# sj-shoff/ImageProcessor

Hardware: AMD Instinct MI355X
Metric: images/sec (resize+thumb+watermark) on 1080p batch at 1/2/4/8 MI355X (higher is better)
Workload: dtype f32+f64

## Files before the change

imageprocessor_amd/build.py:

```python
import concurrent.futures as cf
import os
import subprocess
import sys

HERE = os.path.dirname(os.path.abspath(__file__))
CSRC = os.path.join(HERE, "csrc")
OBJ = os.path.join(HERE, "build")
LIB = os.path.join(HERE, "libipx.so")
SOURCES = ["ipx_kernels.hip", "ipx_ks_generic.hip", "ipx_ks_fused.hip", "ipx_ks_tail.hip", "ipx_jpeg.hip", "ipx_jpeg_entropy.hip", "ipx_jpeg_dec.hip", "ipx_jpeg_dec_par.hip", "ipx_runtime.hip", "ipx_jpeg_runtime.hip", "ipx_pool.hip", "ipx_gif.hip", "ipx_gif_dec.hip", "ipx_png.hip", "ipx_png_dec.hip", "ipx_host.cpp", "ipx_ks_host.cpp", "ipx_batcher.cpp", "ipx_ops.cpp", "ipx_font.cpp", "ipx_jpeg_host.cpp", "ipx_jpeg_dec_host.cpp", "ipx_jpeg_dec_prog.cpp", "ipx_gif_host.cpp", "ipx_gif_dec_host.cpp", "ipx_png_host.cpp", "ipx_png_dec_host.cpp"]
HEADERS = ["ipx_internal.h", "ipx_runtime_internal.h", "ipx_device.h", "ipx_ks.h", "ipx_ks_exact.h", "ipx_threads.h", "ipx_batcher.h", "ipx_pool_core.h", "ipx_gif.h", "ipx_gif_dec.h", "ipx_png.h", "ipx_png_dec.h", os.path.join("..", "..", "include", "ipx.h")]
FLAGS = ["-O3", "-std=c++17", "-fPIC", "--offload-arch=gfx950", "-ffp-contract=off",
         "-fno-fast-math", "-Wall", "-Wno-unused-function"] + os.environ.get("IPX_CXXFLAGS", "").split()


def hipcc():
    for c in (os.environ.get("HIPCC"), "/opt/rocm/bin/hipcc", "hipcc"):
        if c and (os.path.isabs(c) and os.path.exists(c) or not os.path.isabs(c)):
            return c
    return "hipcc"


def sources():
    return [f for f in SOURCES if os.path.exists(os.path.join(CSRC, f))]


def _obj(src):
    return os.path.join(OBJ, src + ".o")


def _newest_header():
    return max(os.path.getmtime(os.path.join(CSRC, h)) for h in HEADERS if os.path.exists(os.path.join(CSRC, h)))


def _stale_objects(force):
    hdr = _newest_header()
    out = []
    for f in sources():
        o = _obj(f)
        if force or not os.path.exists(o) or os.path.getmtime(o) < max(hdr, os.path.getmtime(os.path.join(CSRC, f))):
            out.append(f)
    return out


def stale():
    if not os.path.exists(LIB):
        return True
    t = os.path.getmtime(LIB)
    return any(os.path.getmtime(os.path.join(CSRC, f)) > t for f in sources() + HEADERS if os.path.exists(os.path.join(CSRC, f)))


def build(force=False, verbose=False, jobs=None):
    if not force and not stale():
        return LIB
    os.makedirs(OBJ, exist_ok=True)
    todo = _stale_objects(force)

    def compile_one(f):
        cmd = [hipcc()] + FLAGS + ["-c", "-o", _obj(f), os.path.join(CSRC, f)]
        if verbose:
            print(" ".join(cmd), flush=True)
        subprocess.check_call(cmd)

    jobs = jobs or max(1, min(len(todo), (os.cpu_count() or 2)))
    if todo:
        with cf.ThreadPoolExecutor(jobs) as ex:
            list(ex.map(compile_one, todo))
    cmd = [hipcc(), "-shared", "-fPIC", "--offload-arch=gfx950", "-o", LIB] + [_obj(f) for f in sources()]
    if verbose:
        print(" ".join(cmd), flush=True)
    subprocess.check_call(cmd)
    return LIB


if __name__ == "__main__":
    build(force="--force" in sys.argv, verbose=True)
    print(LIB)
```

imageprocessor_amd/csrc/ipx_ks.h:

```cpp
#pragma once

#include <vector>

#include "ipx_internal.h"

namespace ipx {

struct KsAxis {
    int dw = 0, sw = 0;
    int ntap = 0;
    std::vector<int32_t> lo, cnt;
    std::vector<double> w;
    std::vector<double> itw, itwffff;
    std::vector<double> ones;
};
bool ks_build_axis(int dw, int sw, KsAxis *out);

struct KsAxisDev {
    const int32_t *lo, *cnt;
    const double *w, *itw, *itwffff, *ones;
    int ntap;
};
size_t ks_axis_bytes(const KsAxis &a);
void ks_axis_pack(const KsAxis &a, uint8_t *h, const uint8_t *d, KsAxisDev *out);

enum {
    IPX_SRC_RGBA_CROP = 8,
    IPX_SRC_NRGBA_CROP = 9,
    IPX_SRC_YCBCR_CROP = 10,
    IPX_SRC_TAP64_CROP = 11
};
inline int ks_crop_kind(int kind)
{
    return kind == IPX_SRC_NRGBA ? IPX_SRC_NRGBA_CROP : kind == IPX_SRC_YCBCR ? IPX_SRC_YCBCR_CROP : kind == IPX_SRC_TAP64 ? IPX_SRC_TAP64_CROP
                                                                                                                           : IPX_SRC_RGBA_CROP;
}

struct KsGenArgs {
    uint8_t *dst; int dstride; size_t dst_fs;
    int dr_x0, dr_y0;
    int adr_x0, adr_y0, adr_x1, adr_y1;
    int sr_x0, sr_y0;
    KsAxisDev ax, ay;
    int op;
    const int *opaque_flag;
    int kind;
    const uint8_t *src; int sstride; size_t src_fs;
    const uint8_t *cb, *cr; int cstride, ratio; size_t c_fs;
    int nframes;
    int src_w;
};
hipError_t launch_ks_generic(const KsGenArgs &a, hipStream_t s);

}

namespace ipx {

struct KsStrip { int c0, c1, t0, tw; };
struct KsSeg { int ys, r0, r1; };
template <int NACC> struct KsRowT { double w[NACC], itw[NACC], ones[NACC]; int32_t emit[NACC]; float wf[NACC]; };
static_assert(sizeof(KsRowT<2>) == 64 && sizeof(KsRowT<4>) == 128, "row entries are copied dword-wise");

struct KsFusedOut {
    uint8_t *out; size_t frame_stride; int ostride, obytes;
    int dw, dh, sr_x0, sr_y0;
    int kind;
    int mode, aone;
    int pk;
    int ntap;
    int waves, cpl;
    int wcols;
    const double *wx;
    const float *wxf;
    int split, ntapf;
    float feps;
    const double *itwf;
    const int32_t *xlo;
    const int32_t *colb;
    const void *rows;
    const int32_t *rowoff;
};
struct KsFusedArgs {
    const uint8_t *src; size_t src_fs; int sstride, sw, sh;
    int src_kind;
    int taps_le_alpha;
    const uint8_t *cb, *cr; int cstride, ratio; size_t c_fs;
    uint8_t *wm; size_t wm_fs; int wm_stride;
    int nframes, nstrips, nseg, nthreads, pitch, dbuf;
    const KsStrip *strips; const KsSeg *segs;
    int nout; KsFusedOut o[2];
    int lds_w[2], lds_rows, lds_open;
    int open_per_wave;
    uint8_t wave_role[16];
    unsigned long long *stamps;
    int *redo;
    uint2 *fix; int *fix_count; int fix_cap[2], fix_stride;
};
struct KsText { const DevGlyph *gl; int n; Rect bbox; uint32_t sr, sg, sb, sa; };
struct KsFix { uint2 *list = nullptr; int *count = nullptr; int cap[2] = {0, 0}; KsAxisDev ax[2], ay[2]; };
struct KsFusedGeom { int nseg = 0; const KsSeg *segs = nullptr; const void *rows[2] = {nullptr, nullptr}; const int32_t *rowoff[2] = {nullptr, nullptr}; };
struct KsFusedPlan {
    bool ok = false;
    int nacc = 2, rows = 4, pitch = 0, nstrips = 0, nthreads = 0, nstg = 0, dbuf = 0;
    int lds_w[2] = {0, 0}, lds_rows = 0, lds_open = 0, lds_bytes = 0;
    struct Lds { int dbuf = 0, lds_w[2] = {0, 0}, lds_rows = 0, lds_open = 0, open_per_wave = 0, lds_bytes = 0; } fast;
    const KsStrip *strips = nullptr;
    struct Out { int ntap = 0, waves = 0, cpl = 0, wcols = 0; const double *wx = nullptr, *itwf = nullptr; const int32_t *xlo = nullptr, *colb = nullptr;
                 const float *wxf = nullptr; float feps = 0; int split = 1, ntapf = 0; } o[2];
    KsFusedGeom whole, split;
};
constexpr int kKsSplitRows = 96;
constexpr int kKsRows = 4;
constexpr int kKsMaxStage = 3;
constexpr int kKsMaxWaves = 12;
constexpr int kKsMaxThreads = 64 * kKsMaxWaves;
constexpr int kKsMaxCpl = 2;
constexpr int kKsSplitTaps = 16;
constexpr int kKsOpenPerWave = 128;
struct KsFusedIn { int dw, dh, sr_x0, sr_y0; const KsAxis *hx, *hy; int top_taps = 0; };
bool ks_fused_plan(int sw, int sh, const KsFusedIn *sc0, const KsFusedIn *sc1, int px_bytes, std::vector<uint8_t> *blob, KsFusedPlan *out);
void ks_fused_rebase(KsFusedPlan *p, const uint8_t *dev_blob);
hipError_t launch_ks_fused(const KsFusedPlan &p, KsFusedArgs &a, const KsFix *fix, const KsText *text, int cus, hipStream_t s, bool *matched, bool *text_done);
hipError_t launch_ks_fix(const KsGenArgs &g, const uint2 *list, size_t list_stride, const int *count, int count_stride, int cap, hipStream_t s);

struct KsTailArgs {
    KsGenArgs g[2];
    const uint2 *list[2]; const int *count[2]; int cap[2];
    size_t list_stride; int count_stride;
    int nframes;
    int R[2], chunks[2];
    uint8_t *wm; int wm_stride; size_t wm_fs;
    KsText text;
    int tbx, tby;
};
hipError_t launch_ks_tail(KsTailArgs t, hipStream_t s);

}
```

imageprocessor_amd/csrc/ipx_ks_tail.hip:

```cpp
#include <algorithm>
#include <cstdlib>

#include "ipx_ks_exact.h"

namespace ipx {
namespace {

constexpr int kTailThreads = 256;
constexpr int kTextRows = 4;

template <int KIND>
__device__ __forceinline__ void tail_exact(KsGenArgs a, const uint2 *list, size_t list_stride, const int *count, int count_stride, int cap, int R,
                                           int frame, int chunk, int chunks)
{
    const int n = min(count[(size_t)frame * count_stride], cap);
    list += (size_t)frame * list_stride;
    a.dst += frame * a.dst_fs;
    a.src += frame * a.src_fs;
    if (KIND == IPX_SRC_YCBCR || KIND == IPX_SRC_YCBCR_CROP) { a.cb += frame * a.c_fs; a.cr += frame * a.c_fs; }
    const int lane = (int)threadIdx.x & 63, wv = (int)threadIdx.x >> 6;
    const int per_wave = 64 / R, sub = lane / R, sl = lane - sub * R, per_block = (kTailThreads >> 6) * per_wave;
    ks_exact_list<KIND>(a, list, n, chunk * per_block, chunks * per_block, wv * per_wave + sub, R, sub, sl);
}

__device__ __forceinline__ void tail_text(const KsTailArgs &t, DevGlyph *tab, int f, int rb)
{
    const int by = rb / t.tbx, bx = rb - by * t.tbx;
    const Rect bbox = t.text.bbox;
    const int n = t.text.n;
    const int x = bbox.x0 + bx * 64 + ((int)threadIdx.x & 63);
    const int ybase = bbox.y0 + by * (4 * kTextRows) + ((int)threadIdx.x >> 6);
    uint8_t *frame = t.wm + (size_t)f * t.wm_fs;
    uint32_t d[kTextRows][1], d0[kTextRows];
#pragma unroll
    for (int r = 0; r < kTextRows; r++) {
        const int y = ybase + 4 * r;
        d0[r] = d[r][0] = x < bbox.x1 && y < bbox.y1 ? *(const uint32_t *)(frame + (size_t)y * t.wm_stride + (size_t)x * 4) : 0u;
    }
    for (int g = (int)threadIdx.x; g < n; g += kTailThreads) tab[g] = t.text.gl[g];
    __syncthreads();
    glyph_walk<1, kTextRows, 4>(tab, n, x, ybase, bbox, d, t.text.sr, t.text.sg, t.text.sb, t.text.sa);
#pragma unroll
    for (int r = 0; r < kTextRows; r++) {
        const int y = ybase + 4 * r;
        if (x < bbox.x1 && y < bbox.y1 && d[r][0] != d0[r]) *(uint32_t *)(frame + (size_t)y * t.wm_stride + (size_t)x * 4) = d[r][0];
    }
}

template <int K0, int K1>
__global__ __launch_bounds__(kTailThreads) void ks_tail_kernel(KsTailArgs t)
{
    __shared__ DevGlyph tab[kMaxGlyphs];
    const int nx = t.chunks[0] + t.chunks[1], per = nx + t.tbx * t.tby, b = (int)blockIdx.x;
    const int frame = b / per, c = b - frame * per;
    if (c < nx) {
        const int k = c >= t.chunks[0] ? 1 : 0, chunk = c - (k ? t.chunks[0] : 0);
        if (K0 == K1 || k == 0)
            tail_exact<K0>(k ? t.g[1] : t.g[0], t.list[k], t.list_stride, t.count[k], t.count_stride, t.cap[k], t.R[k], frame, chunk, t.chunks[k]);
        else
            tail_exact<K1>(t.g[1], t.list[1], t.list_stride, t.count[1], t.count_stride, t.cap[1], t.R[1], frame, chunk, t.chunks[1]);
        return;
    }
    tail_text(t, tab, frame, c - nx);
}

template <int K0, int K1>
void tail_go(const KsTailArgs &t, unsigned blocks, hipStream_t s)
{
    hipLaunchKernelGGL((ks_tail_kernel<K0, K1>), dim3(blocks), dim3(kTailThreads), 0, s, t);
}

template <int S, int C>
bool tail_pair(int k0, int k1, const KsTailArgs &t, unsigned blocks, hipStream_t s)
{
    if (k0 == S && k1 == S) tail_go<S, S>(t, blocks, s);
    else if (k0 == S && k1 == C) tail_go<S, C>(t, blocks, s);
    else if (k0 == C && k1 == C) tail_go<C, C>(t, blocks, s);
    else return false;
    return true;
}

}

hipError_t launch_ks_tail(KsTailArgs t, hipStream_t s)
{
    if (t.nframes <= 0) return hipSuccess;
    const char *ev = getenv("IPX_KS_TAIL_BLOCKS");
    const int budget = ev && atoi(ev) > 0 ? atoi(ev) : 2048;
    for (int k = 0; k < 2; k++) {
        t.R[k] = 8; t.chunks[k] = 0;
        if (!t.list[k] || t.cap[k] <= 0) { t.cap[k] = 0; continue; }
        const int ntap = t.g[k].ay.ntap;
        t.R[k] = ntap <= 4 ? 4 : ntap <= 8 ? 8 : ntap <= 16 ? 16 : 64;
        const int per_block = (kTailThreads / 64) * (64 / t.R[k]), most = (t.cap[k] + per_block - 1) / per_block;
        t.chunks[k] = std::max(1, std::min(most, std::max(1, budget / t.nframes)));
    }
    const bool text = t.wm && t.text.gl && t.text.n > 0 && !t.text.bbox.empty();
    if (!text) t.text.n = 0;
    t.tbx = text ? (t.text.bbox.dx() + 63) / 64 : 0;
    t.tby = text ? (t.text.bbox.dy() + 4 * kTextRows - 1) / (4 * kTextRows) : 0;
    const long long blocks = (long long)t.nframes * (t.chunks[0] + t.chunks[1]) + (long long)t.nframes * t.tbx * t.tby;
    if (blocks <= 0) return hipSuccess;
    if (blocks > 0x7fffffffLL) return hipErrorInvalidValue;
    const int k0 = t.chunks[0] ? t.g[0].kind : t.g[1].kind, k1 = t.chunks[1] ? t.g[1].kind : k0;
    const bool none = !t.chunks[0] && !t.chunks[1];
    if (none) { tail_go<IPX_SRC_RGBA, IPX_SRC_RGBA>(t, (unsigned)blocks, s); return hipGetLastError(); }
    if (!tail_pair<IPX_SRC_RGBA, IPX_SRC_RGBA_CROP>(k0, k1, t, (unsigned)blocks, s) && !tail_pair<IPX_SRC_NRGBA, IPX_SRC_NRGBA_CROP>(k0, k1, t, (unsigned)blocks, s) &&
        !tail_pair<IPX_SRC_YCBCR, IPX_SRC_YCBCR_CROP>(k0, k1, t, (unsigned)blocks, s) && !tail_pair<IPX_SRC_TAP64, IPX_SRC_TAP64_CROP>(k0, k1, t, (unsigned)blocks, s))
        return hipErrorInvalidValue;
    return hipGetLastError();
}

}
```

imageprocessor_amd/csrc/ipx_runtime.hip:

```cpp
#include <algorithm>
#include <chrono>
#include <condition_variable>
#include <cstdlib>
#include <cstring>
#include <map>
#include <mutex>
#include <new>
#include <thread>
#include <utility>
#include <vector>

#include "ipx_runtime_internal.h"
#include "ipx_ks.h"

#ifndef IPX_DIAG
#define IPX_DIAG 0
#endif

namespace {

struct ScalePrep {
    bool empty;
    Rect adr;
};
// ... 47 lines not shown
    int cstride = 0, ratio = 0;
    int w = 0, h = 0;
    int nframes = 1;
    size_t frame_stride = 0, c_frame_stride = 0;
    bool le_alpha = false;
};

int dev_draw_src(hipStream_t s, uint8_t *dst, int dw, int dh, int dstride, Rect r, const DevSrc &src, int spx,
                 int spy, int op, size_t dst_fs = 0)
{
    if (op != IPX_OP_OVER && op != IPX_OP_SRC) { set_error("draw: unknown op %d", op); return IPX_ERR_INVALID; }
    int mx = 0, my = 0;
    if (!draw_clip(r, dw, dh, true, src.w, src.h, spx, spy, false, 0, 0, mx, my)) return IPX_OK;
    uint8_t *d = dst + (size_t)r.y0 * dstride + (size_t)r.x0 * 4;
    if (src.kind == IPX_SRC_YCBCR)
        IPX_HIP(launch_draw_ycbcr(d, dstride, src.pix, src.stride, src.cb, src.cr, src.cstride, src.ratio, spx, spy,
                                  r.dx(), r.dy(), s, src.nframes, dst_fs, src.frame_stride, src.c_frame_stride));
    else if (src.kind == IPX_SRC_NRGBA)
        IPX_HIP(launch_draw_nrgba(d, dstride, src.pix + (size_t)spy * src.stride + (size_t)spx * 4, src.stride, r.dx(),
                                  r.dy(), op, s, src.nframes, dst_fs, src.frame_stride));
    else if (src.kind == IPX_SRC_TAP64)
        IPX_HIP(launch_draw_tap64(d, dstride, src.pix + (size_t)spy * src.stride + (size_t)spx * 8, src.stride, r.dx(), r.dy(), op, s,
                                  src.nframes, dst_fs, src.frame_stride));
    else
        for (int i = 0; i < std::max(1, src.nframes); i++)
            IPX_HIP(launch_draw(d + (size_t)i * dst_fs, dstride, src.pix + (size_t)i * src.frame_stride + (size_t)spy * src.stride + (size_t)spx * 4,
                                src.stride, r.dx(), r.dy(), op, s));
    return IPX_OK;
}

int dev_scale_src(ipx_ctx *ctx, hipStream_t s, int *flag, uint8_t *dst, int dw, int dh, int dstride, const Rect &dr,
                  const DevSrc &src, const Rect &sr, int op, size_t dst_fs = 0, int kind_override = -1, const KsAxisDev *axes = nullptr)
{
    ScalePrep pr;
    int rc = scale_prepare(dw, dh, dr, src.w, src.h, sr, op, &pr);
    if (rc) return rc;
    if (pr.empty) return IPX_OK;
    if (src.kind == IPX_SRC_YCBCR) op = IPX_OP_SRC;
    if (op == IPX_OP_OVER && src.kind == IPX_SRC_TAP64) IPX_HIP(launch_opaque_scan_tap64(src.pix, src.w, src.h, src.stride, flag, s));
    else if (op == IPX_OP_OVER) IPX_HIP(launch_opaque_scan(src.pix, src.w, src.h, src.stride, flag, s));
    KsGenArgs a{};
    if (axes) { a.ax = axes[0]; a.ay = axes[1]; }
    else {
        if ((rc = ks_axis_get(ctx, dr.dx(), sr.dx(), &a.ax))) return rc;
        if ((rc = ks_axis_get(ctx, dr.dy(), sr.dy(), &a.ay))) return rc;
    }
    a.dst = dst; a.dstride = dstride; a.src = src.pix; a.sstride = src.stride;
    a.dr_x0 = dr.x0; a.dr_y0 = dr.y0;
    a.adr_x0 = pr.adr.x0; a.adr_y0 = pr.adr.y0; a.adr_x1 = pr.adr.x1; a.adr_y1 = pr.adr.y1;
    a.sr_x0 = sr.x0; a.sr_y0 = sr.y0;
    a.op = op; a.opaque_flag = op == IPX_OP_OVER ? flag : nullptr;
    a.kind = kind_override >= 0 ? kind_override : src.kind;
    a.cb = src.cb; a.cr = src.cr; a.cstride = src.cstride; a.ratio = src.ratio;
    a.nframes = src.nframes; a.src_fs = src.frame_stride; a.c_fs = src.c_frame_stride; a.dst_fs = dst_fs;
    IPX_HIP(launch_ks_generic(a, s));
    return IPX_OK;
}

DevSrc rgba_src(const uint8_t *p, int w, int h, int stride, int kind = IPX_SRC_RGBA)
{
    DevSrc d;
    d.kind = kind; d.pix = p; d.stride = stride; d.w = w; d.h = h;
    return d;
}

int dev_draw(hipStream_t s, uint8_t *dst, int dw, int dh, int dstride, Rect r, const uint8_t *src,
             int sw, int sh, int sstride, int spx, int spy, int op)
{
    return dev_draw_src(s, dst, dw, dh, dstride, r, rgba_src(src, sw, sh, sstride), spx, spy, op);
}

int dev_scale(ipx_ctx *ctx, hipStream_t s, int *flag, uint8_t *dst, int dw, int dh, int dstride, const Rect &dr,
              const uint8_t *src, int sw, int sh, int sstride, const Rect &sr, int op)
{
    return dev_scale_src(ctx, s, flag, dst, dw, dh, dstride, dr, rgba_src(src, sw, sh, sstride), sr, op);
}

int glyphs_for_frame(const ipx_glyphset *gs, int dw, int dh, ClippedGlyphs *out)
{
    std::lock_guard<std::mutex> lk(gs->mu);
    auto it = gs->clipped.find({dw, dh});
    if (it != gs->clipped.end()) { *out = it->second; return IPX_OK; }
    std::vector<DevGlyph> tab;
    Rect bb{0, 0, 0, 0};
    for (const GlyphHost &g : gs->g) {
        Rect r = g.dr;
        int spx = 0, spy = 0, mpx = g.mpx, mpy = g.mpy;
        if (!draw_clip(r, dw, dh, false, 0, 0, spx, spy, true, g.mw, g.mh, mpx, mpy)) continue;
        DevGlyph d;
        d.mask = gs->masks_dev + g.mask_off + (size_t)mpy * g.mw + mpx;
        d.mstride = g.mw;
        d.x0 = r.x0; d.y0 = r.y0; d.x1 = r.x1; d.y1 = r.y1;
        if (tab.empty()) bb = r;
        else {
            bb.x0 = std::min(bb.x0, r.x0); bb.y0 = std::min(bb.y0, r.y0);
            bb.x1 = std::max(bb.x1, r.x1); bb.y1 = std::max(bb.y1, r.y1);
        }
        tab.push_back(d);
    }
    ClippedGlyphs c;
    c.n = (int)tab.size();
    c.bbox = bb;
    if (c.n) {
        IPX_HIP(hipMalloc((void **)&c.dev, tab.size() * sizeof(DevGlyph)));
        IPX_HIP(hipMemcpy(c.dev, tab.data(), tab.size() * sizeof(DevGlyph), hipMemcpyHostToDevice));
    }
    gs->clipped[{dw, dh}] = c;
    *out = c;
    return IPX_OK;
}

int dev_composite(hipStream_t s, uint8_t *dst, int dw, int dh, int dstride, size_t frame_stride,
                  int nframes, const ipx_glyphset *gs)
{
    ClippedGlyphs c;
    int rc = glyphs_for_frame(gs, dw, dh, &c);
    if (rc) return rc;
    IPX_HIP(launch_composite(dst, dstride, frame_stride, nframes, c.dev, c.n, c.bbox,
                             gs->col[0] * 0x101u, gs->col[1] * 0x101u, gs->col[2] * 0x101u,
                             gs->col[3] * 0x101u, s));
    return IPX_OK;
}

}

extern "C" {

static void prepare_hip_env();
int ipx_device_count(void) try
{
    prepare_hip_env();
    clear_error();
    int n = 0;
    hipError_t e = hipGetDeviceCount(&n);
    if (e != hipSuccess) { (void)hipGetLastError(); set_error("hipGetDeviceCount: %s", hipGetErrorString(e)); return IPX_ERR_NODEVICE; }
    return n;
}
IPX_CATCH_STATUS

static void prepare_hip_env()
{
    static std::once_flag once;
    std::call_once(once, [] {
        if (!getenv("GPU_MAX_HW_QUEUES")) {
            char v[16];
            snprintf(v, sizeof v, "%d", std::max(8, env_int("IPX_LANES", 5) + 3));
            setenv("GPU_MAX_HW_QUEUES", v, 0);
        }
    });
}

int ipx_create(const ipx_config *cfg, ipx_ctx **out) try
{
    clear_error();
    if (!out) { set_error("ipx_create: null out"); return IPX_ERR_INVALID; }
    *out = nullptr;
    prepare_hip_env();
    int ndev = 0;
    if (hipGetDeviceCount(&ndev) != hipSuccess || ndev <= 0) {
        (void)hipGetLastError();
        set_error("no HIP device visible: the pixel path has no CPU fallback");
        return IPX_ERR_NODEVICE;
    }
    int dev = cfg ? cfg->device : -1;
    if (dev < 0) dev = env_int("IPX_DEVICE", env_int("LOCAL_RANK", 0) % ndev);
    if (dev >= ndev) { set_error("device %d out of range (%d visible)", dev, ndev); return IPX_ERR_INVALID; }
    IPX_HIP(hipSetDevice(dev));
    hipDeviceProp_t prop;
    IPX_HIP(hipGetDeviceProperties(&prop, dev));
    if (strncmp(prop.gcnArchName, "gfx950", 6) != 0) {
        set_error("device %d is %s; libipx carries gfx950 code only", dev, prop.gcnArchName);
        return IPX_ERR_NODEVICE;
    }
    ipx_ctx *c = new (std::nothrow) ipx_ctx;
    if (!c) { set_error("out of memory"); return IPX_ERR_NOMEM; }
    c->device = dev;
    c->cus = prop.multiProcessorCount > 0 ? prop.multiProcessorCount : 256;
    int lanes = cfg && cfg->lanes > 0 ? cfg->lanes : env_int("IPX_LANES", 5);
    c->lane_bytes = cfg && cfg->lane_bytes ? cfg->lane_bytes : (size_t)64 << 20;
    c->host_cache_limit = (size_t)std::max(0, env_int("IPX_HOST_CACHE_MB", 8192)) << 20;
    c->lanes.resize(lanes);
    int prio_lo = 0, prio_hi = 0;
    (void)hipDeviceGetStreamPriorityRange(&prio_lo, &prio_hi);
    hipError_t e = hipSuccess;
    if (c->lanes.size() >= 3) e = hipStreamCreateWithPriority(&c->lanes.back().stream, hipStreamNonBlocking, prio_hi);
    if (e == hipSuccess) e = hipStreamCreateWithFlags(&c->stream, hipStreamNonBlocking);
    for (size_t i = 0; i < c->lanes.size(); i++) {
        Lane &l = c->lanes[i];
// ... 281 lines not shown
    if (hipEventCreate(&ev) != hipSuccess) { (void)hipGetLastError(); set_error("hipEventCreate failed"); return nullptr; }
    return ev;
}

int ipx_event_record(ipx_ctx *ctx, void *event, void *stream) try
{
    IPX_ENTER(ctx);
    if (!event) { set_error("ipx_event_record: null event"); return IPX_ERR_INVALID; }
    IPX_HIP(hipEventRecord((hipEvent_t)event, stream ? (hipStream_t)stream : ctx->stream));
    return IPX_OK;
}
IPX_CATCH_STATUS

int ipx_event_elapsed_ms(ipx_ctx *ctx, void *start, void *stop, float *ms) try
{
    IPX_ENTER(ctx);
    if (!start || !stop || !ms) { set_error("ipx_event_elapsed_ms: bad argument"); return IPX_ERR_INVALID; }
    IPX_HIP(hipEventSynchronize((hipEvent_t)stop));
    IPX_HIP(hipEventElapsedTime(ms, (hipEvent_t)start, (hipEvent_t)stop));
    return IPX_OK;
}
IPX_CATCH_STATUS

void ipx_event_destroy(ipx_ctx *ctx, void *event)
{
    if (!ctx || !event) return;
    (void)hipSetDevice(ctx->device);
    (void)hipEventDestroy((hipEvent_t)event);
}

int ipx_dev_scale_bilinear_rgba8(ipx_ctx *ctx, void *stream, uint8_t *dst, int dw, int dh,
                                 int dstride, ipx_rect dr, const uint8_t *src, int sw, int sh,
                                 int sstride, ipx_rect sr, int op) try
{
    IPX_ENTER(ctx);
    IPX_FRAME("ipx_dev_scale_bilinear_rgba8", "destination", dst, dw, dh, dstride);
    IPX_FRAME("ipx_dev_scale_bilinear_rgba8", "source", src, sw, sh, sstride);
    hipStream_t s = stream ? (hipStream_t)stream : ctx->stream;
    AsyncFree mem{s, {}};
    int *flag = nullptr;
    if (op == IPX_OP_OVER) IPX_HIP(mem.get(&flag, sizeof(int)));
    return dev_scale(ctx, s, flag, dst, dw, dh, dstride, to_rect(dr), src, sw, sh, sstride, to_rect(sr), op);
}
IPX_CATCH_STATUS

int ipx_dev_draw_rgba8(ipx_ctx *ctx, void *stream, uint8_t *dst, int dw, int dh, int dstride,
                       ipx_rect r, const uint8_t *src, int sw, int sh, int sstride, int spx, int spy,
                       int op) try
{
    IPX_ENTER(ctx);
    IPX_FRAME("ipx_dev_draw_rgba8", "destination", dst, dw, dh, dstride);
    IPX_FRAME("ipx_dev_draw_rgba8", "source", src, sw, sh, sstride);
    return dev_draw(stream ? (hipStream_t)stream : ctx->stream, dst, dw, dh, dstride, to_rect(r), src,
                    sw, sh, sstride, spx, spy, op);
}
IPX_CATCH_STATUS

int ipx_glyphset_create(ipx_ctx *ctx, const ipx_glyph *glyphs, int n, const uint8_t col[4],
                        ipx_glyphset **out) try
{
    IPX_ENTER(ctx);
    if (!out || n < 0 || (n && !glyphs) || !col) { set_error("ipx_glyphset_create: bad argument"); return IPX_ERR_INVALID; }
    if (n > kMaxGlyphs) { set_error("ipx_glyphset_create: %d glyphs exceed the limit of %d", n, kMaxGlyphs); return IPX_ERR_UNSUPPORTED; }
    *out = nullptr;
    ipx_glyphset *gs = new (std::nothrow) ipx_glyphset;
    if (!gs) { set_error("out of memory"); return IPX_ERR_NOMEM; }
    gs->device = ctx->device;
    memcpy(gs->col, col, 4);
    std::vector<uint8_t> blob;
    for (int i = 0; i < n; i++) {
        const ipx_glyph &g = glyphs[i];
        if (g.mw < 0 || g.mh < 0 || (g.mw && g.mh && (!g.mask || g.mstride < g.mw))) {
            set_error("ipx_glyphset_create: glyph %d has a bad mask", i);
            delete gs;
            return IPX_ERR_INVALID;
        }
        GlyphHost h;
        h.mask_off = blob.size();
        h.mw = g.mw; h.mh = g.mh; h.dr = to_rect(g.dr); h.mpx = g.mpx; h.mpy = g.mpy;
        for (int y = 0; y < g.mh; y++) blob.insert(blob.end(), g.mask + (size_t)y * g.mstride, g.mask + (size_t)y * g.mstride + g.mw);
        gs->g.push_back(h);
    }
    gs->masks_bytes = blob.size();
    if (!blob.empty()) {
        hipError_t e = hipMalloc((void **)&gs->masks_dev, blob.size());
        if (e == hipSuccess) e = hipMemcpy(gs->masks_dev, blob.data(), blob.size(), hipMemcpyHostToDevice);
        if (e != hipSuccess) {
            set_error("glyph mask upload failed: %s", hipGetErrorString(e));
            ipx_glyphset_destroy(ctx, gs);
            return IPX_ERR_HIP;
        }
    }
    *out = gs;
    return IPX_OK;
}
IPX_CATCH_STATUS

void ipx_glyphset_destroy(ipx_ctx *ctx, ipx_glyphset *gs)
{
    if (!gs) return;
    (void)hipSetDevice(ctx ? ctx->device : gs->device);
    for (auto &kv : gs->clipped) if (kv.second.dev) (void)hipFree(kv.second.dev);
    if (gs->masks_dev) (void)hipFree(gs->masks_dev);
    delete gs;
}

int ipx_dev_composite_glyphs_rgba8(ipx_ctx *ctx, void *stream, uint8_t *dst, int dw, int dh,
                                   int dstride, const ipx_glyphset *gs) try
{
    IPX_ENTER(ctx);
    if (!gs) { set_error("ipx_dev_composite_glyphs_rgba8: bad argument"); return IPX_ERR_INVALID; }
    IPX_FRAME("ipx_dev_composite_glyphs_rgba8", "destination", dst, dw, dh, dstride);
    return dev_composite(stream ? (hipStream_t)stream : ctx->stream, dst, dw, dh, dstride, 0, 1, gs);
}
IPX_CATCH_STATUS

int ipx_scale_bilinear_rgba8(ipx_ctx *ctx, uint8_t *dst, int dw, int dh, int dstride, ipx_rect dr,
                             const uint8_t *src, int sw, int sh, int sstride, ipx_rect sr, int op) try
{
    IPX_ENTER(ctx);
    IPX_FRAME("ipx_scale_bilinear_rgba8", "destination", dst, dw, dh, dstride);
    IPX_FRAME("ipx_scale_bilinear_rgba8", "source", src, sw, sh, sstride);
    ScalePrep pr;
    int rc = scale_prepare(dw, dh, to_rect(dr), sw, sh, to_rect(sr), op, &pr);
    if (rc) return rc;
    if (pr.empty || dw == 0 || dh == 0) return IPX_OK;
    LaneLease lane(ctx);
    const size_t sbytes = align256((size_t)sw * sh * 4), dbytes = align256((size_t)dw * dh * 4);
    rc = lane_reserve(lane.get(), sbytes + dbytes);
    if (rc) return rc;
    uint8_t *dsrc = lane->dev, *ddst = lane->dev + sbytes;
    hipStream_t s = lane->stream;
    if (sw && sh) IPX_HIP(hipMemcpy2DAsync(dsrc, (size_t)sw * 4, src, sstride, (size_t)sw * 4, sh, hipMemcpyHostToDevice, s));
    IPX_HIP(hipMemcpy2DAsync(ddst, (size_t)dw * 4, dst, dstride, (size_t)dw * 4, dh, hipMemcpyHostToDevice, s));
    rc = dev_scale(ctx, s, lane->flag, ddst, dw, dh, dw * 4, to_rect(dr), dsrc, sw, sh, sw * 4, to_rect(sr), op);
    if (rc) { (void)hipStreamSynchronize(s); return rc; }
    IPX_HIP(hipMemcpy2DAsync(dst, dstride, ddst, (size_t)dw * 4, (size_t)dw * 4, dh, hipMemcpyDeviceToHost, s));
    IPX_HIP(hipStreamSynchronize(s));
    return IPX_OK;
}
IPX_CATCH_STATUS

int ipx_draw_rgba8(ipx_ctx *ctx, uint8_t *dst, int dw, int dh, int dstride, ipx_rect r,
                   const uint8_t *src, int sw, int sh, int sstride, int spx, int spy, int op) try
{
    IPX_ENTER(ctx);
    IPX_FRAME("ipx_draw_rgba8", "destination", dst, dw, dh, dstride);
    IPX_FRAME("ipx_draw_rgba8", "source", src, sw, sh, sstride);
    if (op != IPX_OP_OVER && op != IPX_OP_SRC) { set_error("draw: unknown op %d", op); return IPX_ERR_INVALID; }
    if (!dw || !dh || !sw || !sh) return IPX_OK;
    LaneLease lane(ctx);
    const size_t sbytes = align256((size_t)sw * sh * 4), dbytes = align256((size_t)dw * dh * 4);
    int rc = lane_reserve(lane.get(), sbytes + dbytes);
    if (rc) return rc;
    uint8_t *dsrc = lane->dev, *ddst = lane->dev + sbytes;
    hipStream_t s = lane->stream;
    IPX_HIP(hipMemcpy2DAsync(dsrc, (size_t)sw * 4, src, sstride, (size_t)sw * 4, sh, hipMemcpyHostToDevice, s));
    IPX_HIP(hipMemcpy2DAsync(ddst, (size_t)dw * 4, dst, dstride, (size_t)dw * 4, dh, hipMemcpyHostToDevice, s));
    rc = dev_draw(s, ddst, dw, dh, dw * 4, to_rect(r), dsrc, sw, sh, sw * 4, spx, spy, op);
    if (rc) { (void)hipStreamSynchronize(s); return rc; }
    IPX_HIP(hipMemcpy2DAsync(dst, dstride, ddst, (size_t)dw * 4, (size_t)dw * 4, dh, hipMemcpyDeviceToHost, s));
    IPX_HIP(hipStreamSynchronize(s));
    return IPX_OK;
}
IPX_CATCH_STATUS

int ipx_composite_glyphs_rgba8(ipx_ctx *ctx, uint8_t *dst, int dw, int dh, int dstride,
                               const ipx_glyph *glyphs, int n, const uint8_t col[4]) try
{
    IPX_ENTER(ctx);
    if (n < 0 || (n && !glyphs) || !col) { set_error("ipx_composite_glyphs_rgba8: bad argument"); return IPX_ERR_INVALID; }
    IPX_FRAME("ipx_composite_glyphs_rgba8", "destination", dst, dw, dh, dstride);
    if (!n || !dw || !dh) return IPX_OK;
    ipx_glyphset *gs = nullptr;
    int rc = ipx_glyphset_create(ctx, glyphs, n, col, &gs);
    if (rc) return rc;
    {
        LaneLease lane(ctx);
        rc = lane_reserve(lane.get(), align256((size_t)dw * dh * 4));
        hipStream_t s = lane->stream;
        hipError_t e = hipSuccess;
        if (!rc) {
            e = hipMemcpy2DAsync(lane->dev, (size_t)dw * 4, dst, dstride, (size_t)dw * 4, dh, hipMemcpyHostToDevice, s);
            if (e == hipSuccess) rc = dev_composite(s, lane->dev, dw, dh, dw * 4, 0, 1, gs);
            if (e == hipSuccess && !rc)
// ... 376 lines not shown
{
    clear_error();
    if (!plan || !info) { set_error("ipx_plan_query: bad argument"); return IPX_ERR_INVALID; }
    *info = plan->info;
    return IPX_OK;
}
IPX_CATCH_STATUS

}

static hipError_t composite_text(const ipx_plan *pl, uint8_t *wm, size_t wm_frame_stride, int n, hipStream_t s)
{
    if (!wm || pl->glyphs.n <= 0 || !pl->p.glyphs) return hipSuccess;
    const uint8_t *c = pl->p.glyphs->col;
    return launch_composite(wm, pl->p.sw * 4, wm_frame_stride, n, pl->glyphs.dev, pl->glyphs.n, pl->glyphs.bbox, c[0] * 0x101u, c[1] * 0x101u,
                            c[2] * 0x101u, c[3] * 0x101u, s);
}

static int run_dev_any(ipx_ctx *ctx, hipStream_t s, const ipx_plan *pl, int n, const DevSrc &src, uint8_t *resize_out, size_t resize_frame_stride,
                       uint8_t *thumb_out, size_t thumb_frame_stride, uint8_t *wm_out, size_t wm_frame_stride)
{
    const int sw = pl->p.sw, sh = pl->p.sh;
    uint8_t *outs[2] = {pl->sc[0].on ? resize_out : nullptr, pl->sc[1].on ? thumb_out : nullptr};
    const size_t ostr[2] = {resize_frame_stride, thumb_frame_stride};
    uint8_t *wm = pl->p.do_watermark ? wm_out : nullptr;
    for (int k = 0; k < 2; k++)
        if (pl->sc[k].dw <= 0 || pl->sc[k].dh <= 0) outs[k] = nullptr;
    if (!wm && !outs[0] && !outs[1]) return IPX_OK;
    int kinds[2] = {src.kind, pl->p.crop_to_fit ? ks_crop_kind(src.kind) : src.kind};

    const bool gray = src.kind == IPX_SRC_YCBCR && src.cstride == 0;
    const KsFusedPlan &fp = pl->fused[src.kind == IPX_SRC_RGBA ? 0 : gray ? 2 : 1];
    if (fp.ok && env_int("IPX_FUSED", 1)) {
        KsFusedArgs a{};
        a.src = src.pix; a.src_fs = src.frame_stride; a.sstride = src.stride; a.sw = sw; a.sh = sh;
        a.src_kind = src.kind; a.cb = src.cb; a.cr = src.cr; a.cstride = src.cstride; a.ratio = src.ratio; a.c_fs = src.c_frame_stride;
        a.wm = wm; a.wm_fs = wm_frame_stride; a.wm_stride = sw * 4;
        a.nframes = n;
        a.taps_le_alpha = src.le_alpha;
        for (int k = 0; k < 2; k++) {
            if (!outs[k]) continue;
            const PlanScale &ps = pl->sc[k];
            KsFusedOut &o = a.o[a.nout++];
            o.out = outs[k]; o.frame_stride = ostr[k]; o.ostride = ps.dw * 4; o.obytes = ps.dw * ps.dh * 4;
            o.dw = ps.dw; o.dh = ps.dh; o.sr_x0 = ps.sr.x0; o.sr_y0 = ps.sr.y0;
            o.kind = kinds[k]; o.pk = k;
        }
        AsyncFree mem{s, {}};
        int *redo = nullptr;
        KsFix fixv, *fix = nullptr;
        const int max_items = n * fp.nstrips * std::max(fp.whole.nseg, fp.split.nseg);
        const bool spec = src.kind == IPX_SRC_RGBA && env_int("IPX_KS_SPEC", 1);
        const bool fast = (spec || src.kind == IPX_SRC_YCBCR || src.kind == IPX_SRC_NRGBA || (src.kind == IPX_SRC_TAP64 && src.le_alpha)) &&
                          env_int("IPX_KS_FAST", 1) != 0;
        if (spec || fast) {
            const int cap_env = env_int("IPX_KS_FIX_CAP", 0);
            int cap[2] = {0, 0};
            for (int k = 0; k < 2; k++)
                if (fast && outs[k]) cap[k] = cap_env > 0 ? cap_env : (int)std::min<size_t>(std::max<size_t>((size_t)pl->sc[k].dw * pl->sc[k].dh / 96, 256), (size_t)1 << 20);
            const size_t flags = align256((size_t)max_items * sizeof(int)), counts = fast ? align256((size_t)n * 2 * sizeof(int)) : 0;
            IPX_HIP(mem.get(&redo, flags + counts + (size_t)n * (cap[0] + cap[1]) * sizeof(uint2)));
            if (fast) {
                fixv.count = (int *)((uint8_t *)redo + flags);
                fixv.list = (uint2 *)((uint8_t *)redo + flags + counts);
                fixv.cap[0] = cap[0]; fixv.cap[1] = cap[1];
                for (int k = 0; k < 2; k++) { fixv.ax[k] = pl->sc[k].ax[0]; fixv.ay[k] = pl->sc[k].ax[1]; }
                IPX_HIP(hipMemsetAsync(fixv.count, 0, (size_t)n * 2 * sizeof(int), s));
                fix = &fixv;
            }
        }
        a.redo = redo;
#if IPX_DIAG
        static unsigned long long *stamp_buf = nullptr;
        if (env_int("IPX_STAMPS", 0)) {
            if (!stamp_buf) IPX_HIP(hipMalloc((void **)&stamp_buf, 24 * sizeof(unsigned long long)));
            IPX_HIP(hipMemsetAsync(stamp_buf, 0, 24 * sizeof(unsigned long long), s));
            a.stamps = stamp_buf;
        }
#endif
        KsText text{}, *txt = nullptr;
        if (wm && pl->glyphs.n > 0 && pl->p.glyphs) {
            const uint8_t *c = pl->p.glyphs->col;
            text = KsText{pl->glyphs.dev, pl->glyphs.n, pl->glyphs.bbox, c[0] * 0x101u, c[1] * 0x101u, c[2] * 0x101u, c[3] * 0x101u};
            txt = &text;
        }
        bool matched = false, text_done = false;
        hipError_t e = launch_ks_fused(fp, a, fix, txt, ctx->cus, s, &matched, &text_done);
        if (fix && matched && e == hipSuccess && env_int("IPX_KS_STATS", 0)) {
            std::vector<int> cnt((size_t)n * 2), flags((size_t)max_items);
            (void)hipMemcpyAsync(cnt.data(), fixv.count, cnt.size() * sizeof(int), hipMemcpyDeviceToHost, s);
            (void)hipMemcpyAsync(flags.data(), redo, flags.size() * sizeof(int), hipMemcpyDeviceToHost, s);
            (void)hipStreamSynchronize(s);
            long long tot[2] = {0, 0}; int mx[2] = {0, 0}, nredo = 0;
            for (int i = 0; i < n; i++) for (int k = 0; k < 2; k++) { tot[k] += cnt[2 * i + k]; mx[k] = std::max(mx[k], cnt[2 * i + k]); }
            for (int f : flags) nredo += f != 0;
            fprintf(stderr, "[ipx ks stats] %d frames: undecided pixels per frame resize mean %.1f max %d (room %d), thumbnail mean %.1f max %d (room %d); %d of %d items redone in float64\n", n,
                    (double)tot[0] / n, mx[0], fixv.cap[0], (double)tot[1] / n, mx[1], fixv.cap[1], nredo, max_items);
        }
#if IPX_DIAG
        if (a.stamps && matched) {
            unsigned long long h[24];
            IPX_HIP(hipMemcpyAsync(h, a.stamps, sizeof h, hipMemcpyDeviceToHost, s));
            IPX_HIP(hipStreamSynchronize(s));
            const char *who[3] = {"resize waves", "thumbnail waves", "idle waves"};
            for (int r = 0; r < 3; r++) {
                double tot = 0;
                for (int i = 0; i < 6; i++) tot += (double)h[r * 8 + i];
                if (tot > 0)
                    fprintf(stderr, "[ipx stamps] %-16s share of wave time: wait-loads %.1f%%  drain %.1f%%  barrier %.1f%%  issue %.1f%%  scaleX %.1f%%  scaleY %.1f%%  (%.3g cycles)\n", who[r],
                            100 * h[r * 8] / tot, 100 * h[r * 8 + 1] / tot, 100 * h[r * 8 + 2] / tot, 100 * h[r * 8 + 3] / tot, 100 * h[r * 8 + 4] / tot, 100 * h[r * 8 + 5] / tot, tot);
            }
        }
#endif
        if (e != hipSuccess) { set_error("one-pass kernel launch failed: %s", hipGetErrorString(e)); return IPX_ERR_HIP; }
        if (matched) {
            if (!text_done) IPX_HIP(composite_text(pl, wm, wm_frame_stride, n, s));
            return IPX_OK;
        }
    }

    if (wm) {
        const int rc = dev_draw_src(s, wm, sw, sh, sw * 4, Rect{0, 0, sw, sh}, src, 0, 0, IPX_OP_SRC, wm_frame_stride);
        if (rc) return rc;
        IPX_HIP(composite_text(pl, wm, wm_frame_stride, n, s));
    }
    for (int k = 0; k < 2; k++) {
        if (!outs[k]) continue;
        const PlanScale &ps = pl->sc[k];
        const int rc = dev_scale_src(ctx, s, nullptr, outs[k], ps.dw, ps.dh, ps.dw * 4, Rect{0, 0, ps.dw, ps.dh}, src, ps.sr, IPX_OP_SRC, ostr[k],
                                     kinds[k], ps.ax);
        if (rc) return rc;
    }
    return IPX_OK;
}


int src_check(const char *who, const ipx_plan *pl, const BatchSrc &b, int n, bool in_hbm)
{
    if (b.type < 0 || b.type >= kSrcTypes) { set_error("%s: unknown source type", who); return IPX_ERR_INVALID; }
    const int bpp = src_bpp(b.type);
    bool ok = pl && n >= 0 && b.plane[0] && (long long)b.stride[0] >= (long long)pl->p.sw * bpp;
    if (ok && b.type == kSrcYCbCr) {
        int cw = 0, ch = 0;
        chroma_size(b.ratio, pl->p.sw, pl->p.sh, &cw, &ch);
        ok = b.plane[1] && b.plane[2] && b.ratio >= 0 && b.ratio <= IPX_YCBCR_440 && b.stride[1] >= cw;
    }
    if (ok && b.type == kSrcPaletted) ok = b.palettes && !(in_hbm && ((uintptr_t)b.palettes & 3));
    if (ok && in_hbm && b.type >= kSrcNRGBA64)
        ok = !(((uintptr_t)b.plane[0] | (uintptr_t)b.stride[0] | b.frame_stride[0]) & (b.type == kSrcCMYK ? 3 : 1));
    if (!ok) { set_error("%s: bad argument", who); return IPX_ERR_INVALID; }
    const int sw = pl->p.sw, sh = pl->p.sh;
    if (!frame_span_ok(sw, sh, b.stride[0], bpp) || (b.type == kSrcYCbCr && !frame_span_ok(sw, sh, b.stride[1], 1)) ||
        (b.type >= kSrcNRGBA64 && !frame_span_ok(sw, sh, (long long)sw * 8, 8))) {
        set_error("%s: %dx%d frames with row strides of %d / %d bytes are beyond the 2 GiB span the kernels address", who, sw, sh, b.stride[0], b.stride[1]);
        return IPX_ERR_UNSUPPORTED;
    }
    if (in_hbm && n > 65535) { set_error("%s: at most 65535 frames per call", who); return IPX_ERR_UNSUPPORTED; }
    return IPX_OK;
}

SrcLayout src_layout(const ipx_plan *pl, const BatchSrc &b, size_t (*frame_rule)(size_t))
{
    SrcLayout L{};
    int cw = 0, ch = 0;
    if (b.type == kSrcYCbCr) chroma_size(b.ratio, pl->p.sw, pl->p.sh, &cw, &ch);
    L.planes = b.type == kSrcYCbCr ? 3 : 1;
    L.row[0] = (size_t)pl->p.sw * src_bpp(b.type); L.h[0] = pl->p.sh; L.fs[0] = frame_rule(L.row[0] * L.h[0]);
    L.row[1] = cw; L.h[1] = ch; L.fs[1] = frame_rule((size_t)cw * ch);
    L.pal = b.type == kSrcPaletted ? 1024 : 0;
    return L;
}

hipError_t src_upload(const BatchSrc &host, const SrcLayout &L, int i0, int m, uint8_t *scratch, int slots, hipStream_t s, const CopyPolicy &cp,
                      BatchSrc *in_hbm)
{
    *in_hbm = host;
    hipError_t e = hipSuccess;
    uint8_t *d = scratch;
    for (int p = 0; p < L.planes && e == hipSuccess; p++) {
        const int k = p ? 1 : 0;
// ... 381 lines not shown
```

imageprocessor_amd/csrc/ipx_runtime_internal.h:

```cpp
#pragma once

#include <sched.h>

#include <algorithm>
#include <cctype>
#include <cstdio>
#include <condition_variable>
#include <cstdlib>
#include <cstring>
#include <deque>
#include <map>
#include <mutex>
#include <string>
#include <utility>
#include <vector>

#include "ipx_internal.h"
#include "ipx_ks.h"

using namespace ipx;

struct Lane {
    hipStream_t stream = nullptr;
    uint8_t *dev = nullptr;
    size_t dev_bytes = 0;
    int *flag = nullptr;
    uint8_t *dec = nullptr;
    size_t dec_bytes = 0;
    uint8_t *pin = nullptr;
    size_t pin_bytes = 0;
    hipEvent_t ev[3] = {nullptr, nullptr, nullptr};
    bool busy = false;
};

struct ipx_ctx {
    int device = 0;
    int cus = 256;
    hipStream_t stream = nullptr;
    std::vector<Lane> lanes;
    size_t lane_bytes = 0;
    std::mutex mu;
    std::condition_variable cv;
    std::mutex host_mu;
    std::map<void *, size_t> host_size;
    std::multimap<size_t, void *> host_free_blocks;
    std::deque<void *> host_lru;
    size_t host_cached = 0, host_cache_limit = (size_t)8 << 30;
    int jj_active = 0;
    uint8_t *flat_chroma = nullptr;
    std::mutex plan_mu;
    std::map<std::string, std::pair<ipx_glyphset *, ipx_plan *>> plan_cache;
    uint64_t plan_clock = 0;
    std::mutex ks_mu;
    std::map<std::pair<int, int>, std::pair<uint8_t *, KsAxisDev>> ks_axes;
    static constexpr size_t kFlatChromaBytes = (size_t)64 << 10;
};

struct GlyphHost {
    size_t mask_off;
    int mw, mh;
    Rect dr;
    int mpx, mpy;
};

struct ClippedGlyphs {
    DevGlyph *dev = nullptr;
    int n = 0;
    Rect bbox{0, 0, 0, 0};
};

struct ipx_glyphset {
    int device = 0;
    std::vector<GlyphHost> g;
    uint8_t *masks_dev = nullptr;
    size_t masks_bytes = 0;
    uint8_t col[4] = {0, 0, 0, 0};
    mutable std::mutex mu;
    mutable std::map<std::pair<int, int>, ClippedGlyphs> clipped;
};

struct PlanScale {
    bool on = false;
    int dw = 0, dh = 0;
    Rect sr{0, 0, 0, 0};
    KsAxis hx, hy;
    KsAxisDev ax[2]{};
};

struct ipx_plan {
    ipx_plan_params p{};
    ipx_plan_info info{};
    PlanScale sc[2];
    KsFusedPlan fused[3];
    uint8_t *blob = nullptr;
    ClippedGlyphs glyphs;
    mutable std::mutex mu;
    ipx_glyphset *owned_gs = nullptr;
    int cache_refs = 0;
    uint64_t cache_stamp = 0;
};

inline int env_int(const char *name, int dflt)
{
    const char *v = getenv(name);
    return v && *v ? atoi(v) : dflt;
}

struct DeviceGuard {
    explicit DeviceGuard(int dev) { ok = hipSetDevice(dev) == hipSuccess; }
    bool ok;
};

#define IPX_ENTER(ctx)                                                         \
    clear_error();                                                             \
    if (!(ctx)) { set_error("%s: null context", __func__); return IPX_ERR_INVALID; } \
    DeviceGuard guard_((ctx)->device);                                         \
    if (!guard_.ok) { set_error("hipSetDevice(%d) failed", (ctx)->device); return IPX_ERR_HIP; }

class LaneLease {
public:
    explicit LaneLease(ipx_ctx *c) : c_(c)
    {
        std::unique_lock<std::mutex> lk(c->mu);
        c->cv.wait(lk, [&] {
            for (auto &l : c->lanes) if (!l.busy) return true;
            return false;
        });
        for (auto &l : c->lanes) if (!l.busy) { l.busy = true; lane_ = &l; break; }
    }
    ~LaneLease()
    {
        {
            std::lock_guard<std::mutex> lk(c_->mu);
            lane_->busy = false;
        }
        c_->cv.notify_all();
    }
    Lane *operator->() { return lane_; }
    Lane &get() { return *lane_; }
private:
    ipx_ctx *c_;
    Lane *lane_ = nullptr;
};

inline int lane_reserve_dec(Lane &l, size_t bytes)
{
    if (bytes <= l.dec_bytes) return IPX_OK;
    if (l.dec) { IPX_HIP(hipStreamSynchronize(l.stream)); IPX_HIP(hipFree(l.dec)); l.dec = nullptr; l.dec_bytes = 0; }
    const size_t want = bytes + bytes / 8;
    hipError_t e = hipMalloc((void **)&l.dec, want);
    if (e != hipSuccess) {
        (void)hipGetLastError();
        set_error("device allocation of %zu bytes failed: %s", want, hipGetErrorString(e));
        return IPX_ERR_NOMEM;
    }
    l.dec_bytes = want;
// ... 190 lines not shown
```

Before: 247,900.

## Precompose watermark glyph masks into a per-pixel coverage map for the tail kernel

At glyph-clip time, the host now rasterizes every clipped glyph mask into a dense 16-bit map over the text bounding box, holding up to two overlapping coverage bytes per pixel, and uploads it to the device. The tail kernel's text blocks then read one map entry per pixel and apply at most two glyph_over blends, instead of walking the glyph table per block. This removes per-pixel glyph searching and overlap checks in exchange for an extra map read per pixel and some host-side build memory. It falls back to the old walk when three glyphs overlap a pixel or the box is too large, and it can be disabled with IPX_TEXT_MAP=0.

```diff
diff --git a/imageprocessor_amd/build.py b/imageprocessor_amd/build.py
--- a/imageprocessor_amd/build.py
+++ b/imageprocessor_amd/build.py
@@ -7,8 +7,8 @@
 CSRC = os.path.join(HERE, "csrc")
 OBJ = os.path.join(HERE, "build")
 LIB = os.path.join(HERE, "libipx.so")
-SOURCES = ["ipx_kernels.hip", "ipx_ks_generic.hip", "ipx_ks_fused.hip", "ipx_ks_tail.hip", "ipx_jpeg.hip", "ipx_jpeg_entropy.hip", "ipx_jpeg_dec.hip", "ipx_jpeg_dec_par.hip", "ipx_runtime.hip", "ipx_jpeg_runtime.hip", "ipx_pool.hip", "ipx_gif.hip", "ipx_gif_dec.hip", "ipx_png.hip", "ipx_png_dec.hip", "ipx_host.cpp", "ipx_ks_host.cpp", "ipx_batcher.cpp", "ipx_ops.cpp", "ipx_font.cpp", "ipx_jpeg_host.cpp", "ipx_jpeg_dec_host.cpp", "ipx_jpeg_dec_prog.cpp", "ipx_gif_host.cpp", "ipx_gif_dec_host.cpp", "ipx_png_host.cpp", "ipx_png_dec_host.cpp"]
-HEADERS = ["ipx_internal.h", "ipx_runtime_internal.h", "ipx_device.h", "ipx_ks.h", "ipx_ks_exact.h", "ipx_threads.h", "ipx_batcher.h", "ipx_pool_core.h", "ipx_gif.h", "ipx_gif_dec.h", "ipx_png.h", "ipx_png_dec.h", os.path.join("..", "..", "include", "ipx.h")]
+SOURCES = ["ipx_kernels.hip", "ipx_ks_generic.hip", "ipx_ks_fused.hip", "ipx_ks_tail.hip", "ipx_jpeg.hip", "ipx_jpeg_entropy.hip", "ipx_jpeg_dec.hip", "ipx_jpeg_dec_par.hip", "ipx_runtime.hip", "ipx_jpeg_runtime.hip", "ipx_pool.hip", "ipx_gif.hip", "ipx_gif_dec.hip", "ipx_png.hip", "ipx_png_dec.hip", "ipx_host.cpp", "ipx_ks_host.cpp", "ipx_textmap.cpp", "ipx_batcher.cpp", "ipx_ops.cpp", "ipx_font.cpp", "ipx_jpeg_host.cpp", "ipx_jpeg_dec_host.cpp", "ipx_jpeg_dec_prog.cpp", "ipx_gif_host.cpp", "ipx_gif_dec_host.cpp", "ipx_png_host.cpp", "ipx_png_dec_host.cpp"]
+HEADERS = ["ipx_internal.h", "ipx_runtime_internal.h", "ipx_device.h", "ipx_ks.h", "ipx_ks_exact.h", "ipx_textmap.h", "ipx_threads.h", "ipx_batcher.h", "ipx_pool_core.h", "ipx_gif.h", "ipx_gif_dec.h", "ipx_png.h", "ipx_png_dec.h", os.path.join("..", "..", "include", "ipx.h")]
 FLAGS = ["-O3", "-std=c++17", "-fPIC", "--offload-arch=gfx950", "-ffp-contract=off",
          "-fno-fast-math", "-Wall", "-Wno-unused-function"] + os.environ.get("IPX_CXXFLAGS", "").split()
 
diff --git a/imageprocessor_amd/csrc/ipx_ks.h b/imageprocessor_amd/csrc/ipx_ks.h
--- a/imageprocessor_amd/csrc/ipx_ks.h
+++ b/imageprocessor_amd/csrc/ipx_ks.h
@@ -96,7 +96,7 @@
     int *redo;
     uint2 *fix; int *fix_count; int fix_cap[2], fix_stride;
 };
-struct KsText { const DevGlyph *gl; int n; Rect bbox; uint32_t sr, sg, sb, sa; };
+struct KsText { const DevGlyph *gl; int n; Rect bbox; uint32_t sr, sg, sb, sa; const uint16_t *map = nullptr; int map_pitch = 0, map_depth = -1; };
 struct KsFix { uint2 *list = nullptr; int *count = nullptr; int cap[2] = {0, 0}; KsAxisDev ax[2], ay[2]; };
 struct KsFusedGeom { int nseg = 0; const KsSeg *segs = nullptr; const void *rows[2] = {nullptr, nullptr}; const int32_t *rowoff[2] = {nullptr, nullptr}; };
 struct KsFusedPlan {
diff --git a/imageprocessor_amd/csrc/ipx_ks_tail.hip b/imageprocessor_amd/csrc/ipx_ks_tail.hip
--- a/imageprocessor_amd/csrc/ipx_ks_tail.hip
+++ b/imageprocessor_amd/csrc/ipx_ks_tail.hip
@@ -47,6 +47,33 @@
     }
 }
 
+__device__ __forceinline__ void tail_text_map(const KsTailArgs &t, int f, int rb)
+{
+    const int by = rb / t.tbx, bx = rb - by * t.tbx;
+    const Rect bbox = t.text.bbox;
+    const int x = bbox.x0 + bx * 64 + ((int)threadIdx.x & 63);
+    const int ybase = bbox.y0 + by * (4 * kTextRows) + ((int)threadIdx.x >> 6);
+    uint8_t *frame = t.wm + (size_t)f * t.wm_fs;
+    const uint16_t *map = t.text.map + (x - bbox.x0);
+    uint32_t d0[kTextRows], m[kTextRows];
+#pragma unroll
+    for (int r = 0; r < kTextRows; r++) {
+        const int y = ybase + 4 * r;
+        const bool in = x < bbox.x1 && y < bbox.y1;
+        d0[r] = in ? *(const uint32_t *)(frame + (size_t)y * t.wm_stride + (size_t)x * 4) : 0u;
+        m[r] = in ? (uint32_t)map[(size_t)(y - bbox.y0) * t.text.map_pitch] : 0u;
+    }
+#pragma unroll
+    for (int r = 0; r < kTextRows; r++) {
+        const int y = ybase + 4 * r;
+        const uint32_t lo = m[r] & 0xffu, hi = m[r] >> 8;
+        uint32_t d = d0[r];
+        if (lo) d = glyph_over(d, lo, t.text.sr, t.text.sg, t.text.sb, t.text.sa);
+        if (hi) d = glyph_over(d, hi, t.text.sr, t.text.sg, t.text.sb, t.text.sa);
+        if (d != d0[r]) *(uint32_t *)(frame + (size_t)y * t.wm_stride + (size_t)x * 4) = d;
+    }
+}
+
 template <int K0, int K1>
 __global__ __launch_bounds__(kTailThreads) void ks_tail_kernel(KsTailArgs t)
 {
@@ -61,7 +88,8 @@
             tail_exact<K1>(t.g[1], t.list[1], t.list_stride, t.count[1], t.count_stride, t.cap[1], t.R[1], frame, chunk, t.chunks[1]);
         return;
     }
-    tail_text(t, tab, frame, c - nx);
+    if (t.text.map) tail_text_map(t, frame, c - nx);
+    else tail_text(t, tab, frame, c - nx);
 }
 
 template <int K0, int K1>
@@ -96,7 +124,7 @@
         t.chunks[k] = std::max(1, std::min(most, std::max(1, budget / t.nframes)));
     }
     const bool text = t.wm && t.text.gl && t.text.n > 0 && !t.text.bbox.empty();
-    if (!text) t.text.n = 0;
+    if (!text) { t.text.n = 0; t.text.map = nullptr; }
     t.tbx = text ? (t.text.bbox.dx() + 63) / 64 : 0;
     t.tby = text ? (t.text.bbox.dy() + 4 * kTextRows - 1) / (4 * kTextRows) : 0;
     const long long blocks = (long long)t.nframes * (t.chunks[0] + t.chunks[1]) + (long long)t.nframes * t.tbx * t.tby;
diff --git a/imageprocessor_amd/csrc/ipx_runtime.hip b/imageprocessor_amd/csrc/ipx_runtime.hip
--- a/imageprocessor_amd/csrc/ipx_runtime.hip
+++ b/imageprocessor_amd/csrc/ipx_runtime.hip
@@ -153,11 +153,13 @@
     auto it = gs->clipped.find({dw, dh});
     if (it != gs->clipped.end()) { *out = it->second; return IPX_OK; }
     std::vector<DevGlyph> tab;
+    std::vector<TextMapGlyph> host;
     Rect bb{0, 0, 0, 0};
     for (const GlyphHost &g : gs->g) {
         Rect r = g.dr;
         int spx = 0, spy = 0, mpx = g.mpx, mpy = g.mpy;
         if (!draw_clip(r, dw, dh, false, 0, 0, spx, spy, true, g.mw, g.mh, mpx, mpy)) continue;
+        host.push_back(TextMapGlyph{gs->masks_host.data() + g.mask_off + (size_t)mpy * g.mw + mpx, g.mw, r.x0, r.y0, r.x1, r.y1});
         DevGlyph d;
         d.mask = gs->masks_dev + g.mask_off + (size_t)mpy * g.mw + mpx;
         d.mstride = g.mw;
@@ -175,6 +177,21 @@
     if (c.n) {
         IPX_HIP(hipMalloc((void **)&c.dev, tab.size() * sizeof(DevGlyph)));
         IPX_HIP(hipMemcpy(c.dev, tab.data(), tab.size() * sizeof(DevGlyph), hipMemcpyHostToDevice));
+        std::vector<uint16_t> map;
+        int pitch = 0;
+        const int depth = build_text_map(host.data(), c.n, bb.x0, bb.y0, bb.x1, bb.y1, &map, &pitch);
+        if (depth >= 0) {
+            hipError_t e = hipMalloc((void **)&c.map, map.size() * sizeof(uint16_t));
+            if (e == hipSuccess) e = hipMemcpy(c.map, map.data(), map.size() * sizeof(uint16_t), hipMemcpyHostToDevice);
+            if (e != hipSuccess) {
+                (void)hipGetLastError();
+                if (c.map) (void)hipFree(c.map);
+                (void)hipFree(c.dev);
+                set_error("text map upload failed: %s", hipGetErrorString(e));
+                return IPX_ERR_HIP;
+            }
+            c.map_pitch = pitch; c.map_depth = depth;
+        }
     }
     gs->clipped[{dw, dh}] = c;
     *out = c;
@@ -622,9 +639,10 @@
         gs->g.push_back(h);
     }
     gs->masks_bytes = blob.size();
-    if (!blob.empty()) {
-        hipError_t e = hipMalloc((void **)&gs->masks_dev, blob.size());
-        if (e == hipSuccess) e = hipMemcpy(gs->masks_dev, blob.data(), blob.size(), hipMemcpyHostToDevice);
+    gs->masks_host.swap(blob);
+    if (!gs->masks_host.empty()) {
+        hipError_t e = hipMalloc((void **)&gs->masks_dev, gs->masks_host.size());
+        if (e == hipSuccess) e = hipMemcpy(gs->masks_dev, gs->masks_host.data(), gs->masks_host.size(), hipMemcpyHostToDevice);
         if (e != hipSuccess) {
             set_error("glyph mask upload failed: %s", hipGetErrorString(e));
             ipx_glyphset_destroy(ctx, gs);
@@ -640,7 +658,10 @@
 {
     if (!gs) return;
     (void)hipSetDevice(ctx ? ctx->device : gs->device);
-    for (auto &kv : gs->clipped) if (kv.second.dev) (void)hipFree(kv.second.dev);
+    for (auto &kv : gs->clipped) {
+        if (kv.second.dev) (void)hipFree(kv.second.dev);
+        if (kv.second.map) (void)hipFree(kv.second.map);
+    }
     if (gs->masks_dev) (void)hipFree(gs->masks_dev);
     delete gs;
 }
@@ -1183,6 +1204,7 @@
         if (wm && pl->glyphs.n > 0 && pl->p.glyphs) {
             const uint8_t *c = pl->p.glyphs->col;
             text = KsText{pl->glyphs.dev, pl->glyphs.n, pl->glyphs.bbox, c[0] * 0x101u, c[1] * 0x101u, c[2] * 0x101u, c[3] * 0x101u};
+            if (pl->glyphs.map && env_int("IPX_TEXT_MAP", 1) != 0) { text.map = pl->glyphs.map; text.map_pitch = pl->glyphs.map_pitch; text.map_depth = pl->glyphs.map_depth; }
             txt = &text;
         }
         bool matched = false, text_done = false;
@@ -1197,6 +1219,11 @@
             for (int f : flags) nredo += f != 0;
             fprintf(stderr, "[ipx ks stats] %d frames: undecided pixels per frame resize mean %.1f max %d (room %d), thumbnail mean %.1f max %d (room %d); %d of %d items redone in float64\n", n,
                     (double)tot[0] / n, mx[0], fixv.cap[0], (double)tot[1] / n, mx[1], fixv.cap[1], nredo, max_items);
+        }
+        if (txt && e == hipSuccess && env_int("IPX_KS_STATS", 0)) {
+            if (matched && text_done && text.map) fprintf(stderr, "[ipx text] map %dx%d depth %d\n", text.map_pitch, text.bbox.dy(), text.map_depth);
+            else fprintf(stderr, "[ipx text] walk (%s)\n", !matched ? "no one-pass kernel" : !text_done ? "no tail launch" : pl->glyphs.map ? "IPX_TEXT_MAP=0" :
+                         "no map: three glyphs on a pixel, or a box too large");
         }
 #if IPX_DIAG
         if (a.stamps && matched) {
diff --git a/imageprocessor_amd/csrc/ipx_runtime_internal.h b/imageprocessor_amd/csrc/ipx_runtime_internal.h
--- a/imageprocessor_amd/csrc/ipx_runtime_internal.h
+++ b/imageprocessor_amd/csrc/ipx_runtime_internal.h
@@ -17,6 +17,7 @@
 
 #include "ipx_internal.h"
 #include "ipx_ks.h"
+#include "ipx_textmap.h"
 
 using namespace ipx;
 
@@ -67,11 +68,14 @@
     DevGlyph *dev = nullptr;
     int n = 0;
     Rect bbox{0, 0, 0, 0};
+    uint16_t *map = nullptr;
+    int map_pitch = 0, map_depth = -1;
 };
 
 struct ipx_glyphset {
     int device = 0;
     std::vector<GlyphHost> g;
+    std::vector<uint8_t> masks_host;
     uint8_t *masks_dev = nullptr;
     size_t masks_bytes = 0;
     uint8_t col[4] = {0, 0, 0, 0};
diff --git a/imageprocessor_amd/csrc/ipx_textmap.cpp b/imageprocessor_amd/csrc/ipx_textmap.cpp
--- /dev/null
+++ b/imageprocessor_amd/csrc/ipx_textmap.cpp
@@ -0,0 +1,40 @@
+#include "ipx_textmap.h"
+
+#include <cstddef>
+
+namespace ipx {
+
+int build_text_map(const TextMapGlyph *g, int n, int bx0, int by0, int bx1, int by1, std::vector<uint16_t> *map, int *pitch)
+{
+    map->clear();
+    *pitch = 0;
+    if (n < 0 || (n && !g) || bx1 <= bx0 || by1 <= by0) return -1;
+    const long long w = (long long)bx1 - bx0, h = (long long)by1 - by0;
+    const long long p = (w + kTextMapPitchAlign - 1) / kTextMapPitchAlign * kTextMapPitchAlign;
+    if (p * h > kTextMapMaxPixels) return -1;
+    for (int i = 0; i < n; i++) {
+        const TextMapGlyph &G = g[i];
+        if (G.x1 <= G.x0 || G.y1 <= G.y0) continue;
+        if (G.x0 < bx0 || G.y0 < by0 || G.x1 > bx1 || G.y1 > by1 || !G.mask) return -1;
+    }
+    map->assign((size_t)(p * h), 0);
+    int depth = 0;
+    for (int i = 0; i < n; i++) {
+        const TextMapGlyph &G = g[i];
+        for (int y = G.y0; y < G.y1; y++) {
+            const uint8_t *m = G.mask + (ptrdiff_t)(y - G.y0) * G.mstride;
+            uint16_t *row = map->data() + (size_t)(y - by0) * (size_t)p + (size_t)(G.x0 - bx0);
+            for (int x = 0; x < G.x1 - G.x0; x++) {
+                const uint16_t v = m[x];
+                if (!v) continue;
+                if (!(row[x] & 0xff)) { row[x] = v; if (depth < 1) depth = 1; }
+                else if (!(row[x] >> 8)) { row[x] = (uint16_t)(row[x] | v << 8); depth = 2; }
+                else { map->clear(); return -1; }
+            }
+        }
+    }
+    *pitch = (int)p;
+    return depth;
+}
+
+}
diff --git a/imageprocessor_amd/csrc/ipx_textmap.h b/imageprocessor_amd/csrc/ipx_textmap.h
--- /dev/null
+++ b/imageprocessor_amd/csrc/ipx_textmap.h
@@ -0,0 +1,19 @@
+#pragma once
+
+#include <cstdint>
+#include <vector>
+
+namespace ipx {
+
+struct TextMapGlyph {
+    const uint8_t *mask;
+    int mstride;
+    int x0, y0, x1, y1;
+};
+
+constexpr int kTextMapPitchAlign = 64;
+constexpr long long kTextMapMaxPixels = 1 << 22;
+
+int build_text_map(const TextMapGlyph *g, int n, int bx0, int by0, int bx1, int by1, std::vector<uint16_t> *map, int *pitch);
+
+}
```

Result: faster. 251,200, median of 6 (+1.3%).
